# facebookresearch/robust_cvd

Hardware: AMD Instinct MI355X
Metric: GN/LM iterations/sec (and ms/iter) on 300-frame 384x224 video, 1/2/4/8 GPU (higher is better)
Workload: dtype f64

## Files before the change

include/cvd_hip_debug.h:

```cpp
#ifndef CVD_HIP_DEBUG_H
#define CVD_HIP_DEBUG_H

#include "cvd_hip.h"

#ifdef __cplusplus
extern "C" {
#endif

typedef struct cvd_debug_options {
  uint64_t struct_size;
  int32_t force_iterations;
  int32_t force_sharded_path;
  int32_t pcg_lockstep;
  int32_t stall_fused_tail_once;
  int32_t tail_no_row_staging;
  int32_t tail_closes_scalars;
  int32_t asm_force_stage_depth;
  int32_t asm_force_part_units;
} cvd_debug_options;
void cvd_debug_options_default(cvd_debug_options* o);
int32_t cvd_set_debug_options(cvd_handle* h, const cvd_debug_options* o);

int32_t cvd_set_generic_kernels(cvd_handle* h, int32_t enabled);

int32_t cvd_comm_init_local_group(cvd_handle* h, int32_t rank, int32_t world, uint64_t group_key);
int32_t cvd_comm_init_phantom(cvd_handle* h, int32_t rank, int32_t world);

int32_t cvd_block_inverse_debug(cvd_handle* h, int32_t num_blocks, int32_t block_size, const double* a, int32_t variant,
                                float* inverse, int32_t* failed);

int32_t cvd_epipolar_debug(cvd_handle* h, int32_t num_pairs, const int64_t* offsets, const float* loc, double pixel_scale,
                           double threshold_px, int32_t iterations, uint64_t seed, uint8_t* is_static_out,
                           double* fundamental_out, int32_t* best_out, int32_t* counts_out, double* hypotheses_out);
// ... 15 lines not shown
```

robust_cvd_amd/api.py:

```python
import collections
import ctypes as C
import os
import sys

from . import build as _build
from .binding import Binding
from .ctypes_types import OptParams, SolveSummary, XformDesc

_lib = None
_variant = None


class SolverOptions(C.Structure):
    _fields_ = [
        ("struct_size", C.c_uint64),
        ("pcg_relative_tolerance", C.c_double),
        ("pcg_max_iterations", C.c_int32),
        ("verbose", C.c_int32),
        ("coarse_level", C.c_int32),
        ("robust_loss", C.c_int32),
        ("dense_matrix_free", C.c_int32),
        ("block_inverse_variant", C.c_int32),
        ("coarse_dense_max_unknowns", C.c_int32),
        ("coarse_rebuild_excess", C.c_int32),
# ... 14 lines not shown
        ("temporal_weight", C.c_double),
    ]


class DebugOptions(C.Structure):
    _fields_ = [
        ("struct_size", C.c_uint64),
        ("force_iterations", C.c_int32),
        ("force_sharded_path", C.c_int32),
        ("pcg_lockstep", C.c_int32),
        ("stall_fused_tail_once", C.c_int32),
        ("tail_no_row_staging", C.c_int32),
        ("tail_closes_scalars", C.c_int32),
        ("asm_force_stage_depth", C.c_int32),
        ("asm_force_part_units", C.c_int32),
    ]


class ConsistencyDesc(C.Structure):
    _fields_ = [
        ("struct_size", C.c_uint64),
        ("precision", C.c_int32),
        ("num_frames", C.c_int32),
        ("num_pairs", C.c_int32),
        ("height", C.c_int32),
        ("width", C.c_int32),
        ("distance_type", C.c_int32),
        ("have_warp", C.c_int32),
        ("reserved", C.c_int32),
        ("lambda_reprojection", C.c_double),
# ... 1793 lines not shown
        ai = np.zeros((n, n))
        lam = np.zeros(self.num_frames * self.block_size())
        fl = C.c_int32(0)
        dp = lambda x: x.ctypes.data_as(C.POINTER(C.c_double))
        self._check(self._fn("temporal_debug")(self._h, dims, dp(a), dp(ai), dp(lam), C.byref(fl)))
        return {"NT": n, "S": dims[1], "nn": dims[2], "step": dims[3], "Sx": dims[4], "Sy": dims[5], "a_t": a, "a_t_inverse": ai,
                "lam": lam, "failed": fl.value}

    def path_info(self):
        out = (C.c_int32 * 8)()
        self._check(self._fn("path_info")(self._h, out))
        form = {-1: "none", 0: "exact sparse factor", 1: "exact dense inverse", 2: "temporal pose level"}[out[1]]
        return {"pose_graph_level": form, "depth_grid_level": bool(out[2]), "fused_tail": bool(out[3] & 1), "tail_rows_staged": bool(out[3] & 2),
                "product_sums_shares": bool(out[3] & 4), "rz_shares": out[3] >> 8,
                "tail_disabled": bool(out[4]),
                "taps": out[5], "work_items": out[6], "cross_blocks": bool(out[7])}

    def product_launch_debug(self):
        out = (C.c_int32 * 6)()
        self._check(self._fn("product_launch_debug")(self._h, out))
        kind = {-1: "none", 0: "generic list", 1: "fast list", 2: "fast dense", 3: "cross blocks"}[out[3]]
        return {"threads": out[0], "spec": out[1], "kd": out[2], "kind": out[3], "kind_name": kind, "work_items": out[4],
                "num_cu": out[5]}

    def assembly_launch_debug(self):
        import numpy as np
        out = (C.c_int32 * 8)()
        cost = np.zeros(self.num_frames, dtype=np.float64)
        self._check(self._fn("assembly_launch_debug")(self._h, out, cost.ctypes.data_as(C.POINTER(C.c_double))))
        kind = {-1: "none", 0: "generic", 1: "fast list", 2: "fast dense", 3: "dense fold"}[out[3]]
        return {"threads": out[0], "spec": out[1], "kd": out[2], "kind": out[3], "kind_name": kind, "workgroups": out[4],
# ... 15 lines not shown
```

robust_cvd_amd/csrc/cvd_api.hip:

```cpp
#include "cvd_host.h"
#include "cvd_coarse.h"

namespace cvd {

static void poseOptimizationStep(cvd_handle* h, const cvd_opt_params& p, double depthDeformReg) {
  solve(h, p, depthDeformReg, PK_POSE_STEP);
  paramsToPoses(h, p);
}

static void poseOptimization(cvd_handle* h, const cvd_opt_params& p) {
  posesToParams(h);
  h->records.clear();
  int ctfRows = p.ctf_long, ctfCols = p.ctf_short;
  int dsoRows = p.dso_long, dsoCols = p.dso_short;
  if (h->aspect >= 1.f) {
    std::swap(ctfCols, ctfRows);
    std::swap(dsoCols, dsoRows);
  }
  int initGrid[3] = {1, 1, 1};
  if (h->ddesc.depth_type == CVD_DEPTH_GRID)
    for (int i = 0; i < 3; ++i) initGrid[i] = h->ddesc.grid_size[i];
  const int Nval = (h->ddesc.depth_type == CVD_DEPTH_IDENTITY) ? 0 : valueNumParams(h->ddesc.value_xform);
  size_t nDmax = static_cast<size_t>(h->nD());
  if (p.coarse_to_fine && h->ddesc.depth_type != CVD_DEPTH_IDENTITY && p.num_steps > 1)
// ... 243 lines not shown
      h->tableValid = false;
    if (o->constraint_order != h->opt.constraint_order) h->orderGx = h->orderGy = -1;
    h->opt = *o;
  });
}
void cvd_debug_options_default(cvd_debug_options* o) {
  o->struct_size = CVD_STRUCT_STAMP(cvd_debug_options);
  o->force_iterations = 0;
  o->force_sharded_path = 0;
  o->pcg_lockstep = 0;
  o->stall_fused_tail_once = 0;
  o->tail_no_row_staging = 0;
  o->tail_closes_scalars = 0;
  o->asm_force_stage_depth = 0;
  o->asm_force_part_units = 0;
}
int32_t cvd_set_debug_options(cvd_handle* h, const cvd_debug_options* o) {
  CVD_TRY(h, {
    if (o->struct_size != CVD_STRUCT_STAMP(cvd_debug_options))
      throw std::runtime_error("cvd_debug_options: struct_size does not match this library's cvd_hip_debug.h (start from cvd_debug_options_default)");
    if (o->asm_force_stage_depth < 0 || o->asm_force_stage_depth > 3) throw std::runtime_error("asm_force_stage_depth in {0, 1, 2, 3}");
    if (o->asm_force_part_units < 0) throw std::runtime_error("asm_force_part_units >= 0");
    if (o->asm_force_part_units != h->dbg.asm_force_part_units) h->tableValid = false;
    h->dbg = *o;
    h->distForced = h->world == 1 && (h->comm != nullptr || h->localGroup || h->phantom) && o->force_sharded_path != 0;
  });
}
void cvd_comm_unique_id(uint8_t* out128) {
  ncclUniqueId id;
  std::memset(&id, 0, sizeof(id));
// ... 767 lines not shown
      HIP_CHECK(hipStreamSynchronize(s));
      if (failed) *failed = fl;
    }
  });
}
int32_t cvd_path_info(cvd_handle* h, int32_t* out8) {
  CVD_TRY(h, {
    out8[0] = h->coarseOn ? 1 : 0;
    out8[1] = !h->coarseOn ? -1 : (h->coarse.temporalPose ? 2 : (h->coarse.denseMode ? 1 : 0));
    out8[2] = h->temporal.on ? 1 : 0;
    out8[3] = h->lastFusedTail ? (h->tailStageRows ? 3 : 1) : 0;
    if (h->lastFusedTail && h->lastShares) out8[3] |= 4 | (h->lastShareCount << 8);
    out8[4] = h->tailDisabled ? 1 : 0;
    out8[5] = h->lastKD;
    out8[6] = static_cast<int32_t>(h->itemFa.size());
    out8[7] = h->lastCross ? 1 : 0;
  });
}
int32_t cvd_product_launch_debug(cvd_handle* h, int32_t* out6) {
  CVD_TRY(h, {
    for (int i = 0; i < 6; ++i) out6[i] = h->lastProduct[i];
  });
}
int32_t cvd_assembly_launch_debug(cvd_handle* h, int32_t* out8, double* cost_frame) {
  CVD_TRY(h, {
    for (int i = 0; i < 8; ++i) out8[i] = h->lastAssembly[i];
    const size_t F = static_cast<size_t>(h->F);
    if (cost_frame && h->lastAssembly[3] >= 0 && h->dCostFrame.n >= F) {
      h->dCostFrame.download(cost_frame, F, h->stream);
      HIP_CHECK(hipStreamSynchronize(h->stream));
    }
// ... 80 lines not shown
```

robust_cvd_amd/csrc/cvd_eval.hip:

```cpp
#include "cvd_host.h"
#include "cvd_cost.h"
#include "cvd_assembly.h"
#include "cvd_triplets.h"
#include "cvd_dense_walk.h"

namespace cvd {

void launchFrameConsts(Ctx& c, const double* x) {
  launchFrameConsts(c.L, x, c.h->dFc.p, c.h->stream);
  HIP_CHECK(hipGetLastError());
}

void spinStream(hipStream_t s) {
  hipError_t e;
  while ((e = hipStreamQuery(s)) == hipErrorNotReady) {}
  HIP_CHECK(e);
}
void spinEvent(hipEvent_t ev) {
  hipError_t e;
  while ((e = hipEventQuery(ev)) == hipErrorNotReady) {}
  HIP_CHECK(e);
}
void readScalars(Ctx& c) {
  HIP_CHECK(hipMemcpyAsync(c.h->hScal, c.h->dScal.p, S_COUNT * sizeof(double), hipMemcpyDeviceToHost, c.h->stream));
  spinStream(c.h->stream);
}
// ... 264 lines not shown
```

robust_cvd_amd/csrc/cvd_host.h:

```cpp
#pragma once

#include <hip/hip_runtime.h>
#include <hip/hip_ext.h>
#include <rccl/rccl.h>
#include <rocblas/rocblas.h>
#include <rocsolver/rocsolver.h>

#include <algorithm>
#include <array>
#include <atomic>
#include <chrono>
#include <condition_variable>
#include <cmath>
#include <cstdarg>
#include <cstdint>
#include <cstdio>
#include <cstdlib>
#include <cstring>
#include <functional>
#include <limits>
#include <map>
#include <memory>
#include <mutex>
#include <set>
#include <stdexcept>
#include <string>
#include <thread>
#include <tuple>
#include <vector>

#include "../../include/cvd_hip_debug.h"
#include "cvd_kernels.h"
#include "cvd_asm_segments.h"


namespace cvd {

inline std::string fmt(const char* f, ...) {
  char buf[1024];
  va_list ap;
  va_start(ap, f);
  vsnprintf(buf, sizeof(buf), f, ap);
  va_end(ap);
  return buf;
}

#define HIP_CHECK(expr)                                                                          \
  do {                                                                                           \
// ... 278 lines not shown
    DevBuf<TlStep> stepDev;
    hipEvent_t evIn = nullptr, evDone = nullptr;
    bool sidePending = false;
    double* sqPtr = nullptr;
  } temporal;
  hipEvent_t evRebuild[2] = {nullptr, nullptr};
  bool rebuildTimed = false;
  double coarseRebuildMs = 0.0, pcgIterMs = 0.0;
  std::vector<std::pair<int, int>> globalEdges;
  bool haveGlobalEdges = false;
  DevBuf<double> dRegJac;
  DevBuf<unsigned short> dRegCol;
  DevBuf<unsigned char> dRegCnt;
  RegCache regCache{};
  DevBuf<FrameConst> dFc;
  DevBuf<int> dFail;
  DevBuf<unsigned long long> dCount;
  double* hScal = nullptr;
  double* hStage[2] = {nullptr, nullptr};
  size_t hStageN[2] = {0, 0};
  double* hPcg = nullptr;
  hipEvent_t pcgEvent[2] = {nullptr, nullptr};

  cvd_solve_summary summary{};
  std::vector<cvd_iteration_record> records;

  bool lastFusedTail = false, lastCross = false;
  bool lastShares = false;
  int lastShareCount = 0;
  int sharesF = -1, sharesN = -1;
  bool tailStageRows = false;
  int lastKD = 0;
  int lastProduct[6] = {0, 0, 0, -1, 0, 0};
  int lastAssembly[8] = {0, 0, 0, -1, 0, 0, -1, 0};
  bool tailDisabled = false;
  bool forceGeneric = false;

  int timing = 0;
  int timingStride = 1;
  long long timingCounter = 0;
  long long timingCounterKc[16] = {0};
  std::vector<std::pair<hipEvent_t, hipEvent_t>> evPool;
// ... 195 lines not shown
  ~DenseListScope();
};
bool denseModeSupported(const cvd_opt_params& p, const cvd_xform_desc& dd, const cvd_xform_desc& sd, bool haveTriplets, int world,
                        bool normalize);
AsmPanels makePanels(int B, size_t capDoubles, int& panelCap);
void compileTable(cvd_handle* h, const std::vector<int>& range, bool withTriplets = false, bool ignoreStatic = false);
void orderTable(cvd_handle* h, const Layout& L, int KD);
double* pinnedStage(cvd_handle* h, int which, size_t n);
void uploadState(cvd_handle* h, const Layout& L, DevBuf<double>& dst);
void downloadState(cvd_handle* h, const Layout& L, const DevBuf<double>& src);
void buildMask(cvd_handle* h, const Layout& L, const cvd_opt_params& p, ProblemKind kind, const std::vector<int>& range);
void ensureBuffers(Ctx& c);
void refreshMedians(cvd_handle* h);
void launchFrameConsts(const Layout& L, const double* x, FrameConst* fc, hipStream_t s);
void launchFrameConsts(Ctx& c, const double* x);
void launchFlagToBool(int* flag, hipStream_t s);
void launchTlRowsInit(cvd_handle* h, const TlStep* tsp, int NT, int groups, int F, unsigned int* counter, int closeScalars, double tol2,
                      hipStream_t s);
void spinStream(hipStream_t s);
void spinEvent(hipEvent_t ev);
void readScalars(Ctx& c);
void enqueueCost(Ctx& c, const double* x);
double evalCost(Ctx& c, const double* x);
void enqueueStats(Ctx& c);
bool crossScope(cvd_handle* h, const Ctx& c);
CrossPairs crossPairs(cvd_handle* h);
void launchCrossAssemble(Ctx& c, const double* x);
double evalFull(Ctx& c, const double* x, bool withStats = false, bool noReadBack = false);
bool coarseFusedConsumers();
bool fusedExchange(cvd_handle* h, bool withCoarse);
// ... 20 lines not shown
                  double* q, bool withCoarse = false, bool tailFused = false, int sharesIteration = 0);
bool pcgTailScope(Ctx& c, bool coarse, int nThreads, size_t& lds, int& ldsFinish, int& ldsScratch);
struct PcgShares {
  int count = 0;
  int levelShare0 = 0;
  int levelWg0 = 0;
};
bool pcgSharesScope(Ctx& c, bool coarse, PcgShares& sh);
void launchPcgTail(Ctx& c, const double* x, const double* pOld, double* pNew, int useBeta, const double* lam, double* q,
                   bool withCoarse, int nThreads, size_t lds, int ldsFinish, int ldsScratch, double tol2,
                   const PcgShares* shares = nullptr);
void launchPcgClose(Ctx& c, int enqueued);
void launchBlockInverseRaw(cvd_handle* h, const Layout& L, const double* dH, const double* dLam, float* dMinv, int* dFail, int variant,
                           hipStream_t onStream = nullptr);
void launchBlockInverse(Ctx& c, hipStream_t onStream = nullptr);
void launchCoarseSetup(Ctx& c, const double* x, int side = 0);
bool temporalScope(const Ctx& c);
bool temporalPrepare(Ctx& c);
void launchTemporalSetup(Ctx& c, const double* x, int half);
void launchTemporalInit(Ctx& c, bool closeScalars, double tol2);
TlStep temporalStep(cvd_handle* h);
const TlStep* temporalStepDev(cvd_handle* h);
void poseTemporalPlan(cvd_handle* h);
void poseTemporalPrepare(Ctx& c);
void launchPoseTemporalBuild(Ctx& c, hipStream_t s, int* failOut, bool deferInverse = false);
void launchPoseTemporalInit(Ctx& c, double tol2);
const TlStep* poseTemporalStepDev(cvd_handle* h);
void coarseDebug(cvd_handle* h, int32_t* num_unknowns, double* a_c, double* a_c_inverse, int32_t* failed);
int runPcg(Ctx& c, const double* x, const std::function<void()>& tail = nullptr);
bool wantsTriplets(const cvd_opt_params& p, ProblemKind kind);
void bindTriplets(Ctx& c, const cvd_opt_params& p, ProblemKind kind);
void solve(cvd_handle* h, const cvd_opt_params& p, double depthDeformReg, ProblemKind kind);
void evaluate(cvd_handle* h, const cvd_opt_params& p, double depthDeformReg, const double* pose7, double* cost, int32_t* nres,
              double* gradient, double* hdiag, double* hfull);
// ... 115 lines not shown
```

robust_cvd_amd/csrc/cvd_precond.hip:

```cpp
#include "cvd_host.h"
#include "cvd_block_inverse.h"
#include "cvd_coarse.h"
#include "cvd_cross.h"
#include "cvd_dense_walk.h"
#include "cvd_dense_inverse.h"

namespace cvd {

void launchFlagToBool(int* flag, hipStream_t s) { hipLaunchKernelGGL(k_flag_to_bool, dim3(1), dim3(1), 0, s, flag); }

void launchBlockInverseRaw(cvd_handle* h, const Layout& L, const double* dH, const double* dLam, float* dMinv,
                                  int* dFail, int variant, hipStream_t onStream) {
  hipStream_t s = onStream ? onStream : h->stream;
  const int B = L.B;
  if (B > 256) {
    if (onStream) throw std::logic_error("launchBlockInverseRaw: the rocSOLVER route runs on the solver's stream");
    if (!h->rbMain) {
      if (rocblas_create_handle(&h->rbMain) != rocblas_status_success) throw std::runtime_error("rocblas_create_handle failed");
      if (rocblas_set_stream(h->rbMain, s) != rocblas_status_success) throw std::runtime_error("rocblas_set_stream failed");
    }
    const size_t bb = static_cast<size_t>(B) * B, total = bb * L.F;
    h->dInvScratch.ensure(total);
    h->dInvInfo.ensure(2 * static_cast<size_t>(L.F));
    HIP_CHECK(hipMemsetAsync(h->dInvInfo.p, 0, 2 * static_cast<size_t>(L.F) * sizeof(int), s));
// ... 124 lines not shown
  else if (tpw <= 5) CVD_LAUNCH_DINV(5);
  else if (tpw <= 8) CVD_LAUNCH_DINV(8);
  else if (tpw <= 13) CVD_LAUNCH_DINV(13);
  else if (tpw <= 18) CVD_LAUNCH_DINV(18);
  else CVD_LAUNCH_DINV(25);
#undef CVD_LAUNCH_DINV
  HIP_CHECK(hipGetLastError());
}
void launchDenseSpdInversePair(cvd_handle* h, const DinvRequest& a, const DinvRequest& b, hipStream_t s) {
  const DinvPlan Pa = planDenseSpdInverse(h, a.n, a.A, a.out, a.fail, s, a.outValid, a.panelBuf, a.barrierBuf);
  const DinvPlan Pb = planDenseSpdInverse(h, b.n, b.A, b.out, b.fail, s, b.outValid, b.panelBuf, b.barrierBuf);
  const size_t lds = std::max(Pa.lds, Pb.lds);
  bool pair = Pa.tpw <= 2 && Pb.tpw <= 2 && CVD_DETERMINISTIC == 0;
  if (pair) {
    allowLds((k_dense_spd_inverse_pair<2>), lds);
    int perCu = 0;
    HIP_CHECK(hipOccupancyMaxActiveBlocksPerMultiprocessor(&perCu, reinterpret_cast<const void*>(&k_dense_spd_inverse_pair<2>), kDinvNW * 64, lds));
    pair = static_cast<long long>(perCu) * h->numCU >= 2ll * std::max(Pa.job.groups, Pb.job.groups);
  }
  if (!pair) {
    launchDenseSpdInverse(h, a.n, a.A, a.out, a.fail, s, a.outValid, a.panelBuf, a.barrierBuf);
    launchDenseSpdInverse(h, b.n, b.A, b.out, b.fail, s, b.outValid, b.panelBuf, b.barrierBuf);
    return;
  }
  PersistentGate gate(h->device, s);
  hipLaunchKernelGGL((k_dense_spd_inverse_pair<2>), dim3(std::max(Pa.job.groups, Pb.job.groups), 2), dim3(kDinvNW * 64), lds, s, Pa.job, Pb.job);
  HIP_CHECK(hipGetLastError());
}

void launchCoarseSetup(Ctx& c, const double* x, int side) {
  cvd_handle* h = c.h;
  hipStream_t s = side ? h->stream2 : h->stream;
  auto& C = h->coarse;
  const size_t B = c.L.B;
  double* WbOut = side ? C.Wb2.p : C.Wb.p;
  int* failOut = side ? C.fail2.p : C.fail.p;
  FrameConst* fcBuf = side ? h->dFc2.p : h->dFc.p;
  HIP_CHECK(hipMemsetAsync(failOut, 0, sizeof(int), s));
  {
    launchFrameConsts(c.L, x, fcBuf, s);
    HIP_CHECK(hipMemsetAsync(C.edges.p, 0, static_cast<size_t>(std::max(C.nEdges, 1)) * kCBB * sizeof(double), s));
    if (C.sparsified) HIP_CHECK(hipMemsetAsync(C.dropDiag.p, 0, static_cast<size_t>(c.L.F) * kCBB * sizeof(double), s));
    const size_t ldsE = 2 * B * 8 + 2 * sizeof(FrameConst) + 4 * kCBB * 8;
    if (c.cross && !C.sparsified) {
      hipLaunchKernelGGL(k_coarse_edges_cross, dim3(static_cast<unsigned>(h->xFa.size())), dim3(256), 0, s, c.L, crossPairs(h),
                         h->dXBlocks.p, h->dXPairEdge.p, C.edges.p);
    } else if (c.nItems > 0) {
      const bool fast = !h->forceGeneric && c.KS == 0 && fastLoss(c.L) &&
                        c.L.intrOpt != CVD_INTR_SHARED;
      const bool gram = fast && !h->dense && c.KD == 4 && c.L.N == 1 && !C.sparsified && CVD_DETERMINISTIC == 0;
      if (gram) {
        const size_t ldsG = (2 * B + 512 + 4 * 64 * kDwLd) * 8;
        allowLds(k_coarse_edges_mfma, ldsG);
        hipLaunchKernelGGL(k_coarse_edges_mfma, dim3(c.nItems), dim3(256), ldsG, s, c.L, c.T, c.it, x, fcBuf, C.itemEdgeDev.p, C.edges.p);
      } else if (fast) {
// ... 14 lines not shown
          hipLaunchKernelGGL((k_coarse_edges<KD, KS>), dim3(c.nItems), dim3(256), ldsE, s, c.L, c.T, c.it, x, fcBuf,
                             C.itemEdgeDev.p, C.edges.p, C.dropDiag.p);
        });
      }
    }
    HIP_CHECK(hipGetLastError());
    if (h->dist()) {
      const int ct = h->tBegin(KC_COMM_COARSE);
      commAllReduce(h, C.edges.p, static_cast<size_t>(C.nEdges) * kCBB, CT_F64, s);
      if (C.sparsified)
        commAllReduce(h, C.dropDiag.p, static_cast<size_t>(c.L.F) * kCBB, CT_F64, s);
      h->tEnd(ct);
    }
  }
  constexpr double lamPredict = 1.0 / 3.0;
  hipLaunchKernelGGL(k_coarse_diag, dim3(c.L.F), dim3(256), 0, s, c.L, h->dH.p, h->dLam.p, h->dMask.p, C.diag.p,
                     C.modeActive.p, side ? lamPredict : 1.0, C.sparsified ? C.dropDiag.p : nullptr);
  if (h->dist()) {
    const int ct = h->tBegin(KC_COMM_COARSE);
    const size_t chunk = static_cast<size_t>(h->ownChunk()) * kCBB;
    commAllGather(h, C.diag.p + static_cast<size_t>(h->rank) * chunk, C.diag.p, chunk, CT_F64, s);
    h->tEnd(ct);
  }
  if (C.denseMode) {
    if (side) throw std::logic_error("the dense coarse level is built in line");
    if (C.temporalPose) {
      C.denseValid.ensure(1);
      if (!(C.denseReady && C.denseForB == static_cast<int>(c.L.B))) HIP_CHECK(hipMemsetAsync(C.denseValid.p, 0, sizeof(int), s));
      launchPoseTemporalBuild(c, s, failOut, h->temporal.on && !h->dist());
      if (h->dist()) {
        launchFlagToBool(failOut, s);
        const int ct = h->tBegin(KC_COMM_COARSE);
// ... 46 lines not shown
```

robust_cvd_amd/csrc/cvd_setup.hip:

```cpp
#include "cvd_host.h"
#include "cvd_table.h"
#include "cvd_triplets.h"
#include "cvd_dense_walk.h"
#include <rocprim/device/device_segmented_radix_sort.hpp>

namespace cvd {

void launchFrameConsts(const Layout& L, const double* x, FrameConst* fc, hipStream_t s) {
  hipLaunchKernelGGL(k_frame_consts, dim3((L.F + 63) / 64), dim3(64), 0, s, L, x, fc);
}

static void quatToMatrix(const double q[4] , double R[3][3]) {
  for (int c = 0; c < 3; ++c) {
    double v[3] = {0, 0, 0};
    v[c] = 1.0;
    const double uv[3] = {2.0 * (q[1] * v[2] - q[2] * v[1]), 2.0 * (q[2] * v[0] - q[0] * v[2]),
                          2.0 * (q[0] * v[1] - q[1] * v[0])};
    R[0][c] = v[0] + q[3] * uv[0] + (q[1] * uv[2] - q[2] * uv[1]);
    R[1][c] = v[1] + q[3] * uv[1] + (q[2] * uv[0] - q[0] * uv[2]);
    R[2][c] = v[2] + q[3] * uv[2] + (q[0] * uv[1] - q[1] * uv[0]);
  }
}
static void matrixToAngleAxis(const double R[3][3], double aa[3]) {
  double q0, q1, q2, q3;
// ... 1081 lines not shown
  }
  return h->hStage[which];
}

void uploadState(cvd_handle* h, const Layout& L, DevBuf<double>& dst) {
  const size_t nAll = static_cast<size_t>(L.F) * L.B;
  double* x = pinnedStage(h, 1, nAll);
  const int nD = L.nD, nS = L.nS;
  for (int f = 0; f < L.F; ++f) {
    double* xf = &x[static_cast<size_t>(f) * L.B];
    for (int i = 0; i < 7; ++i) xf[i] = h->poseParams[f][i];
    for (int i = 0; i < nD; ++i) xf[7 + i] = h->dparams[static_cast<size_t>(f) * nD + i];
    for (int i = 0; i < nS; ++i) xf[7 + nD + i] = h->sparams[static_cast<size_t>(f) * nS + i];
  }
  dst.upload(x, nAll, h->stream);
  HIP_CHECK(hipStreamSynchronize(h->stream));
}

void downloadState(cvd_handle* h, const Layout& L, const DevBuf<double>& src) {
  const size_t nAll = static_cast<size_t>(L.F) * L.B;
  double* x = pinnedStage(h, 0, nAll);
  src.download(x, nAll, h->stream);
  HIP_CHECK(hipStreamSynchronize(h->stream));
  const int nD = L.nD, nS = L.nS;
  for (int f = 0; f < L.F; ++f) {
    const double* xf = &x[static_cast<size_t>(f) * L.B];
    for (int i = 0; i < 7; ++i) h->poseParams[f][i] = xf[i];
    for (int i = 0; i < nD; ++i) h->dparams[static_cast<size_t>(f) * nD + i] = xf[7 + i];
    for (int i = 0; i < nS; ++i) h->sparams[static_cast<size_t>(f) * nS + i] = xf[7 + nD + i];
  }
// ... 115 lines not shown
```

robust_cvd_amd/csrc/cvd_solve.hip:

```cpp
#include <optional>

#include "cvd_host.h"
#include "cvd_lm.h"
#include "cvd_pcg.h"
#include "cvd_coarse.h"

namespace cvd {

void launchTlRowsInit(cvd_handle* h, const TlStep* tsp, int NT, int groups, int F, unsigned int* counter, int closeScalars, double tol2,
                      hipStream_t s) {
  const size_t lds = static_cast<size_t>(tlRowsLds(NT)) * 8;
  allowLds(k_tl_rows_init, lds);
  hipLaunchKernelGGL(k_tl_rows_init, dim3(groups), dim3(768), lds, s, tsp, F, h->dScal.p, counter, closeScalars, tol2, h->hPcg);
  HIP_CHECK(hipGetLastError());
}

namespace {
struct TailStalled {};
}
static int runPcgAttempt(Ctx& c, const double* x, const std::function<void()>& tail);
int runPcg(Ctx& c, const double* x, const std::function<void()>& tail) {
  const size_t firstTimerSlot = c.h->evUsed;
  try {
    return runPcgAttempt(c, x, tail);
// ... 312 lines not shown
    }
  }
};

void rebuildTemporalLevel(Ctx& c) {
  cvd_handle* h = c.h;
  const int slot = h->tBegin(KC_INVERSE);
  launchTemporalSetup(c, h->dX.p, 0);
  launchTemporalSetup(c, h->dX.p, 1);
  h->tEnd(slot);
}

void buildLevels(Ctx& c, const LevelSchedule::Decision& d, PendingGuard& guard) {
  cvd_handle* h = c.h;
  hipStream_t s = h->stream;
  if (d.inverseAside) {
    HIP_CHECK(hipEventRecord(h->evInvIn, s));
    HIP_CHECK(hipStreamWaitEvent(h->stream3, h->evInvIn, 0));
    launchBlockInverse(c, h->stream3);
    HIP_CHECK(hipEventRecord(h->evInvDone, h->stream3));
    guard.inverseAside = true;
  } else {
    const int slot = h->tBegin(KC_INVERSE);
    launchBlockInverse(c);
    h->tEnd(slot);
  }
  if (d.coarse == LevelSchedule::SIDE_STREAM) {
    h->dFc2.ensure(c.L.F);
    if (h->temporal.on) rebuildTemporalLevel(c);
    HIP_CHECK(hipEventRecord(h->evCoarseIn, s));
    HIP_CHECK(hipStreamWaitEvent(h->stream2, h->evCoarseIn, 0));
    launchCoarseSetup(c, h->dX.p, 1);
    HIP_CHECK(hipEventRecord(h->evCoarseDone, h->stream2));
  } else if (d.coarse == LevelSchedule::IN_LINE) {
    const int slot = h->tBegin(KC_INVERSE);
    const bool measure = h->coarse.denseMode && !h->dist() && h->opt.coarse_rebuild_excess_dense < 0;
    if (measure) {
      if (!h->evRebuild[0]) for (auto& e : h->evRebuild) HIP_CHECK(hipEventCreate(&e));
      HIP_CHECK(hipEventRecord(h->evRebuild[0], s));
    }
    if (h->temporal.on) launchTemporalSetup(c, h->dX.p, 0);
    launchCoarseSetup(c, h->dX.p);
    if (d.inverseAside) {
      HIP_CHECK(hipStreamWaitEvent(s, h->evInvDone, 0));
      guard.inverseAside = false;
    }
    if (h->temporal.on) launchTemporalSetup(c, h->dX.p, 1);
    if (measure) {
      HIP_CHECK(hipEventRecord(h->evRebuild[1], s));
      h->rebuildTimed = true;
    }
    h->tEnd(slot);
  }
  if (d.temporalOnly) rebuildTemporalLevel(c);
}

void installPendingCoarse(cvd_handle* h, LevelSchedule& schedule) {
// ... 27 lines not shown
  h->records.push_back(rec);
  if (tableLine && h->opt.verbose)
    printf("%4d % .6e    % .2e   % .2e   % .2e  % .2e % .2e   %5d\n", rec.iteration, cost, rec.cost_change, gmax, rec.step_norm,
           rec.relative_decrease, radius, rec.linear_iterations);
}

}

void solve(cvd_handle* h, const cvd_opt_params& p, double depthDeformReg, ProblemKind kind) {
  const double t0 = nowSeconds();
  if (h->F <= 0) throw std::runtime_error("no video set");
  if (!h->poseParamsValid) posesToParams(h);
  const std::vector<int> range = rangeOf(p, h->F);
  LevelSchedule schedule;
  PendingGuard guard{h, schedule};
  SetupPhases phase{h->opt.verbose >= 3};
  BoundProblem bound;
  bindProblem(bound, h, p, depthDeformReg, kind, range, BindMode{ true,  true,  true}, phase);
  Ctx& c = bound.c;
  hipStream_t s = h->stream;
  HIP_CHECK(hipMemsetAsync(h->dDx.p, 0, c.n * sizeof(double), s));
  HIP_CHECK(hipMemsetAsync(h->dR.p, 0, c.n * sizeof(double), s));
  HIP_CHECK(hipMemsetAsync(h->dFail.p, 0, sizeof(int), s));

  cvd_solve_summary sum{};
  sum.num_residual_blocks = static_cast<int>((c.L.includeStatic ? h->numValid : 0) + countResidualBlocks(c, range));
  double tEval = 0.0, tLin = 0.0;
  double te = nowSeconds();
  double xCost = evalFull(c, h->dX.p, true, false);
  tEval += nowSeconds() - te;
// ... 29 lines not shown
      ++iteration;
      cvd_iteration_record rec{};
      rec.iteration = iteration;

      double tl = nowSeconds();
      hipLaunchKernelGGL(k_lm_diag, dim3((c.n + 255) / 256), dim3(256), 0, s, c.L, h->dHd.p, h->dScale.p,
                         scaleDone ? 0 : 1, tr.radius, h->dLam.p);
      scaleDone = true;
      buildLevels(c, schedule.decide(levels), guard);
      const double tPcgStart = nowSeconds();
      const int cgIters = runPcg(c, h->dX.p, [&]() {
        enqueueStats(c);
        hipLaunchKernelGGL(k_apply_step, dim3((c.n + 255) / 256), dim3(256), 0, s, c.L, c.boundDepth0, h->dX.p,
                           h->dDx.p, h->dXc.p);
        HIP_CHECK(hipGetLastError());
        enqueueCost(c, h->dXc.p);
      });
      notePcgTime(h, nowSeconds() - tPcgStart, cgIters);
      schedule.afterPcg(cgIters);
      installPendingCoarse(h, schedule);
      tLin += nowSeconds() - tl;
      if (gradPending) {
        gradPending = false;
        gmax = h->hScal[S_GMAX];
        xNorm = std::sqrt(h->hScal[S_XX]);
        h->records.back().gradient_max_norm = gmax;
        if (gradientConverged()) {
          --iteration;
          termination = 0;
          break;
// ... 129 lines not shown
```

robust_cvd_amd/csrc/cvd_temporal.hip:

```cpp
#include "cvd_host.h"
#include "cvd_temporal.h"

namespace cvd {

static int autoCoarse(int g, int wanted) {
  const int s = wanted > 0 ? wanted : (g + 1) / 2;
  return std::min(g, std::max(2, s));
}

bool temporalScope(const Ctx& c) {
  cvd_handle* h = c.h;
  const Layout& L = c.L;
  if (h->opt.temporal_level == 0 || h->forceGeneric || (h->dense && !c.cross) || c.trip) return false;
  if (c.KD != 4 || c.KS != 0 || !fastLoss(L) || L.intrOpt == CVD_INTR_SHARED) return false;
  if (L.N != 1 || L.gz != 1 || L.depthType != CVD_DEPTH_GRID || L.positionRegSqrt > 0.0 || !L.includeStatic) return false;
  if (L.B > 256 || L.nD > 256 || L.gx < 3 || L.gy < 3 || L.nD != L.gx * L.gy) return false;
  const int step = h->opt.temporal_step;
  if (L.F <= 2 * step) return false;
  const int Sx = autoCoarse(L.gx, h->opt.temporal_grid_x), Sy = autoCoarse(L.gy, h->opt.temporal_grid_y);
  if (Sx * Sy > kTlMaxS) return false;
  const int nn = (L.F - 1 + step - 1) / step + 1;
  if (nn * Sx * Sy > kDenseCoarseMaxUnknowns) return false;
  return true;
}
// ... 148 lines not shown
}

TlStep temporalStep(cvd_handle* h) {
  if (h == nullptr || !h->temporal.on || !h->temporal.built)
    return TlStep{nullptr, nullptr, nullptr, nullptr, nullptr, nullptr, nullptr, nullptr, nullptr, 0, 0, 1, 0, 0, 0, 1, kTlSpan, nullptr, 1.0};
  auto& T = h->temporal;
  return TlStep{T.Ainv.p, T.sqPtr, T.rT.p, T.t.p, T.tl.p, T.dotPart.p, T.fail.p, T.elW.p, T.elV.p, T.S, T.nn, T.step, T.NT, T.NT, T.width,
                tlParts(T.nn), kTlSpan, (!h->dist() && T.step <= 32) ? T.rec.p : nullptr,
                h->opt.temporal_weight};
}

const TlStep* temporalStepDev(cvd_handle* h) {
  return (h != nullptr && h->temporal.on && h->temporal.built) ? h->temporal.stepDev.p : nullptr;
}

void launchTemporalSetup(Ctx& c, const double* x, int half) {
  cvd_handle* h = c.h;
  auto& T = h->temporal;
  const Layout& L = c.L;
  const bool side = !h->dist() && h->stream2 != nullptr;
  hipStream_t s = (half == 0 && side) ? h->stream2 : h->stream;
  if (half == 1) {
    if (side && T.sidePending) {
      HIP_CHECK(hipStreamWaitEvent(h->stream, T.evDone, 0));
      T.sidePending = false;
    }
    temporalInverse(c);
    return;
  }
  const TlTables tb = temporalTables(h);
  const size_t SS = static_cast<size_t>(T.S) * T.S;
  FrameConst* fcBuf = h->dFc.p;
  if (side) {
    if (!T.evIn) {
      HIP_CHECK(hipEventCreateWithFlags(&T.evIn, hipEventDisableTiming));
      HIP_CHECK(hipEventCreateWithFlags(&T.evDone, hipEventDisableTiming));
    }
    h->dFc2.ensure(L.F);
    fcBuf = h->dFc2.p;
    HIP_CHECK(hipEventRecord(T.evIn, h->stream));
    HIP_CHECK(hipStreamWaitEvent(s, T.evIn, 0));
  }
  launchFrameConsts(L, x, fcBuf, s);
  const size_t ldsD = static_cast<size_t>(L.nD) * T.S * 8 + static_cast<size_t>(T.width) * T.S * 5 + 16;
  allowLds(k_tl_diag, ldsD);
  hipLaunchKernelGGL(k_tl_diag, dim3(L.F), dim3(256), ldsD, s, L, h->dH.p, h->dLam.p, h->dMask.p, tb, T.Cf.p,
                     h->dist() ? h->ownFirst() : 0, h->dist() ? h->ownCount() : L.F);
  HIP_CHECK(hipGetLastError());
  if (c.cross) {
    if (!h->xFa.empty()) {
      allowLds(k_tl_edges_cross, ldsD);
      hipLaunchKernelGGL(k_tl_edges_cross, dim3(static_cast<unsigned>(h->xFa.size())), dim3(256), ldsD, s, L, h->dXFa.p, h->dXFb.p,
                         h->dXBlocks.p, h->dMask.p, tb, T.E.p);
      hipLaunchKernelGGL(k_tl_reduce, dim3(T.nGroups), dim3(256), 0, s, T.S, T.step, T.gOff.p, T.gItems.p, h->dXFa.p, h->dXFb.p, T.E.p,
                         T.part.p);
      HIP_CHECK(hipGetLastError());
    }
  } else if (c.nItems > 0) {
    const size_t ldsE = 2 * static_cast<size_t>(L.B) * 8 + 2 * sizeof(FrameConst) + SS * 8 + 3 * static_cast<size_t>(L.gx + L.gy) * 4 + 16;
    allowLds(k_tl_edges<false>, ldsE);
    hipLaunchKernelGGL(k_tl_edges<false>, dim3(c.nItems), dim3(256), ldsE, s, L, c.T, c.it, x, fcBuf, h->dMask.p, tb, T.E.p);
    HIP_CHECK(hipGetLastError());
    hipLaunchKernelGGL(k_tl_reduce, dim3(T.nGroups), dim3(256), 0, s, T.S, T.step, T.gOff.p, T.gItems.p, h->dItemFa.p, h->dItemFb.p,
// ... 179 lines not shown
```

Baseline: 359.1.

## Fuse coarse and temporal per-frame diagonal builds; cache frame constants and occupancy query

Adds a single k_level_diag kernel that reads each frame's Hessian block once and produces both the coarse-level diagonal blocks and the temporal-level Cf blocks, replacing the separate k_coarse_diag and k_tl_diag launches on the single-GPU in-line build path. It also tags the frame-constant buffer with a parameter write generation so that repeated launchFrameConsts calls on unchanged parameters are skipped. A third change memoises the occupancy query for the pair inverse kernel. The fused kernel uses LDS double atomics and 1024-thread workgroups, which makes summation order nondeterministic. The cache depends on every parameter write being noted, so a missed write could leave stale constants.

```diff
diff --git a/include/cvd_hip_debug.h b/include/cvd_hip_debug.h
--- a/include/cvd_hip_debug.h
+++ b/include/cvd_hip_debug.h
@@ -17,6 +17,7 @@
   int32_t tail_closes_scalars;
   int32_t asm_force_stage_depth;
   int32_t asm_force_part_units;
+  int32_t level_build_separate;
 } cvd_debug_options;
 void cvd_debug_options_default(cvd_debug_options* o);
 int32_t cvd_set_debug_options(cvd_handle* h, const cvd_debug_options* o);
diff --git a/robust_cvd_amd/api.py b/robust_cvd_amd/api.py
--- a/robust_cvd_amd/api.py
+++ b/robust_cvd_amd/api.py
@@ -52,6 +52,7 @@
         ("tail_closes_scalars", C.c_int32),
         ("asm_force_stage_depth", C.c_int32),
         ("asm_force_part_units", C.c_int32),
+        ("level_build_separate", C.c_int32),
     ]
 
 
@@ -1875,7 +1876,8 @@
         return {"pose_graph_level": form, "depth_grid_level": bool(out[2]), "fused_tail": bool(out[3] & 1), "tail_rows_staged": bool(out[3] & 2),
                 "product_sums_shares": bool(out[3] & 4), "rz_shares": out[3] >> 8,
                 "tail_disabled": bool(out[4]),
-                "taps": out[5], "work_items": out[6], "cross_blocks": bool(out[7])}
+                "taps": out[5], "work_items": out[6], "cross_blocks": bool(out[7] & 1),
+                "level_build_fused": bool(out[7] & 2)}
 
     def product_launch_debug(self):
         out = (C.c_int32 * 6)()
diff --git a/robust_cvd_amd/csrc/cvd_api.hip b/robust_cvd_amd/csrc/cvd_api.hip
--- a/robust_cvd_amd/csrc/cvd_api.hip
+++ b/robust_cvd_amd/csrc/cvd_api.hip
@@ -281,6 +281,7 @@
   o->tail_closes_scalars = 0;
   o->asm_force_stage_depth = 0;
   o->asm_force_part_units = 0;
+  o->level_build_separate = 0;
 }
 int32_t cvd_set_debug_options(cvd_handle* h, const cvd_debug_options* o) {
   CVD_TRY(h, {
@@ -1078,7 +1079,7 @@
     out8[4] = h->tailDisabled ? 1 : 0;
     out8[5] = h->lastKD;
     out8[6] = static_cast<int32_t>(h->itemFa.size());
-    out8[7] = h->lastCross ? 1 : 0;
+    out8[7] = (h->lastCross ? 1 : 0) | (h->lastLevelBuildFused ? 2 : 0);
   });
 }
 int32_t cvd_product_launch_debug(cvd_handle* h, int32_t* out6) {
diff --git a/robust_cvd_amd/csrc/cvd_eval.hip b/robust_cvd_amd/csrc/cvd_eval.hip
--- a/robust_cvd_amd/csrc/cvd_eval.hip
+++ b/robust_cvd_amd/csrc/cvd_eval.hip
@@ -6,10 +6,21 @@
 
 namespace cvd {
 
+static uint64_t frameConstKey(const Layout& L) {
+  uint64_t f;
+  static_assert(sizeof(f) == sizeof(L.vFocal), "vFocal is a double");
+  std::memcpy(&f, &L.vFocal, sizeof(f));
+  return f ^ (static_cast<uint64_t>(L.F) << 40) ^ (static_cast<uint64_t>(L.B) << 20) ^ (static_cast<uint64_t>(L.intrOpt) << 60);
+}
 void launchFrameConsts(Ctx& c, const double* x) {
-  launchFrameConsts(c.L, x, c.h->dFc.p, c.h->stream);
-  HIP_CHECK(hipGetLastError());
-}
+  cvd_handle* h = c.h;
+  const uint64_t key = frameConstKey(c.L);
+  if (h->fcTag.holds(x, h->dFc.p, key)) return;
+  launchFrameConsts(c.L, x, h->dFc.p, h->stream);
+  HIP_CHECK(hipGetLastError());
+  h->fcTag.filled(x, h->dFc.p, key);
+}
+void noteParamsWritten(cvd_handle* h, const double* x) { h->fcTag.wrote(x); }
 
 void spinStream(hipStream_t s) {
   hipError_t e;
diff --git a/robust_cvd_amd/csrc/cvd_fc_tag.h b/robust_cvd_amd/csrc/cvd_fc_tag.h
--- /dev/null
+++ b/robust_cvd_amd/csrc/cvd_fc_tag.h
@@ -0,0 +1,45 @@
+#pragma once
+
+#include <cstdint>
+
+namespace cvd {
+
+struct FrameConstTag {
+  static constexpr int kBufs = 4;
+  struct Buf {
+    const void* p = nullptr;
+    uint64_t gen = 0;
+  };
+  Buf bufs[kBufs];
+  uint64_t clock = 0;
+  const void* x = nullptr;
+  const void* fc = nullptr;
+  uint64_t gen = 0, key = 0;
+
+  uint64_t generationOf(const void* p) const {
+    for (const Buf& b : bufs)
+      if (b.p == p && p != nullptr) return b.gen;
+    return 0;
+  }
+  void wrote(const void* p) {
+    Buf* slot = &bufs[0];
+    for (Buf& b : bufs) {
+      if (b.p == p) { slot = &b; break; }
+      if (b.gen < slot->gen) slot = &b;
+    }
+    slot->p = p;
+    slot->gen = ++clock;
+  }
+  void filled(const void* xp, const void* fcp, uint64_t k) {
+    x = xp;
+    fc = fcp;
+    key = k;
+    gen = generationOf(xp);
+  }
+  bool holds(const void* xp, const void* fcp, uint64_t k) const {
+    return gen != 0 && xp == x && fcp == fc && k == key && generationOf(xp) == gen;
+  }
+  void invalidate() { gen = 0; }
+};
+
+}
diff --git a/robust_cvd_amd/csrc/cvd_host.h b/robust_cvd_amd/csrc/cvd_host.h
--- a/robust_cvd_amd/csrc/cvd_host.h
+++ b/robust_cvd_amd/csrc/cvd_host.h
@@ -32,6 +32,7 @@
 #include "../../include/cvd_hip_debug.h"
 #include "cvd_kernels.h"
 #include "cvd_asm_segments.h"
+#include "cvd_fc_tag.h"
 
 
 namespace cvd {
@@ -340,6 +341,7 @@
   DevBuf<unsigned char> dRegCnt;
   RegCache regCache{};
   DevBuf<FrameConst> dFc;
+  FrameConstTag fcTag;
   DevBuf<int> dFail;
   DevBuf<unsigned long long> dCount;
   double* hScal = nullptr;
@@ -352,6 +354,7 @@
   std::vector<cvd_iteration_record> records;
 
   bool lastFusedTail = false, lastCross = false;
+  bool lastLevelBuildFused = false;
   bool lastShares = false;
   int lastShareCount = 0;
   int sharesF = -1, sharesN = -1;
@@ -577,6 +580,7 @@
 void refreshMedians(cvd_handle* h);
 void launchFrameConsts(const Layout& L, const double* x, FrameConst* fc, hipStream_t s);
 void launchFrameConsts(Ctx& c, const double* x);
+void noteParamsWritten(cvd_handle* h, const double* x);
 void launchFlagToBool(int* flag, hipStream_t s);
 void launchTlRowsInit(cvd_handle* h, const TlStep* tsp, int NT, int groups, int F, unsigned int* counter, int closeScalars, double tol2,
                       hipStream_t s);
@@ -627,10 +631,12 @@
 void launchBlockInverseRaw(cvd_handle* h, const Layout& L, const double* dH, const double* dLam, float* dMinv, int* dFail, int variant,
                            hipStream_t onStream = nullptr);
 void launchBlockInverse(Ctx& c, hipStream_t onStream = nullptr);
-void launchCoarseSetup(Ctx& c, const double* x, int side = 0);
+void launchCoarseSetup(Ctx& c, const double* x, int side = 0, bool frameBlocksDone = false);
 bool temporalScope(const Ctx& c);
 bool temporalPrepare(Ctx& c);
-void launchTemporalSetup(Ctx& c, const double* x, int half);
+void launchTemporalSetup(Ctx& c, const double* x, int half, bool frameBlocksDone = false);
+bool levelBuildFusedScope(const Ctx& c);
+void launchLevelDiag(Ctx& c, hipStream_t s);
 void launchTemporalInit(Ctx& c, bool closeScalars, double tol2);
 TlStep temporalStep(cvd_handle* h);
 const TlStep* temporalStepDev(cvd_handle* h);
diff --git a/robust_cvd_amd/csrc/cvd_level_build.h b/robust_cvd_amd/csrc/cvd_level_build.h
--- /dev/null
+++ b/robust_cvd_amd/csrc/cvd_level_build.h
@@ -0,0 +1,126 @@
+#pragma once
+
+#include "cvd_temporal.h"
+
+namespace cvd {
+
+constexpr int kLevelDiagThreads = 1024;
+constexpr int kLevelDiagRows = 4;
+constexpr int kLevelDiagChunks = 4;
+
+inline __global__ __launch_bounds__(kLevelDiagThreads) void k_level_diag(Layout L, const double* __restrict__ hBlocks,
+                                                                  const double* __restrict__ lam, const double* __restrict__ mask,
+                                                                  TlTables T, double* __restrict__ diagOut,
+                                                                  unsigned char* __restrict__ modeActive, double* __restrict__ Cf) {
+  extern __shared__ __attribute__((aligned(16))) double sm[];
+  __shared__ int anyScale;
+  constexpr int NT = kLevelDiagThreads, NW = NT / 64;
+  const int B = L.B, G = L.nD, S = T.S, Gs = G | 1, f = blockIdx.x, tid = threadIdx.x, lane = tid & 63;
+  const int wave = __builtin_amdgcn_readfirstlane(tid >> 6);
+  double* T1 = sm;
+  double* u = T1 + static_cast<size_t>(S) * Gs;
+  double* red = u + B;
+  float* ew = reinterpret_cast<float*>(red + NW);
+  unsigned char* ev = reinterpret_cast<unsigned char*>(ew + T.width * S);
+  const double* hf = hBlocks + static_cast<size_t>(f) * B * B;
+  const double* lf = lam + static_cast<size_t>(f) * B;
+  const double* mf = mask + static_cast<size_t>(f) * B;
+  double* out = Cf + static_cast<size_t>(f) * S * S;
+  const bool tlOn = mf[7] != 0.0;
+  if (tid == 0) anyScale = 0;
+  for (int r = tid; r < B; r += NT) u[r] = 0.0;
+  if (tlOn) {
+    for (int e = tid; e < S * Gs; e += NT) T1[e] = 0.0;
+    for (int e = tid; e < T.width * S; e += NT) {
+      ew[e] = T.elW[e];
+      ev[e] = T.elV[e];
+    }
+  }
+  __syncthreads();
+  {
+    bool in[kLevelDiagChunks], grid[kLevelDiagChunks];
+    double lv[kLevelDiagChunks], us[kLevelDiagChunks];
+#pragma unroll
+    for (int j = 0; j < kLevelDiagChunks; ++j) {
+      const int c = lane + 64 * j, v = c - 7;
+      in[j] = c < B;
+      grid[j] = in[j] && v >= 0 && v < G;
+      lv[j] = grid[j] ? lf[c] : 0.0;
+      us[j] = 0.0;
+    }
+    const double* col = hf + static_cast<size_t>(7) * B + lane;
+    for (int vp0 = wave; vp0 < G; vp0 += NW * kLevelDiagRows) {
+      double hv[kLevelDiagRows][kLevelDiagChunks];
+#pragma unroll
+      for (int q = 0; q < kLevelDiagRows; ++q) {
+        const int vp = vp0 + NW * q;
+#pragma unroll
+        for (int j = 0; j < kLevelDiagChunks; ++j) hv[q][j] = (vp < G && in[j]) ? col[static_cast<size_t>(vp) * B + 64 * j] : 0.0;
+      }
+#pragma unroll
+      for (int q = 0; q < kLevelDiagRows; ++q) {
+        const int vp = vp0 + NW * q;
+        if (vp >= G) break;
+        const float4 w = T.vW[vp];
+        const unsigned int idx = T.vIdx[vp];
+#pragma unroll
+        for (int j = 0; j < kLevelDiagChunks; ++j) {
+          const int v = lane + 64 * j - 7;
+          const double h = hv[q][j] + (v == vp ? lv[j] : 0.0);
+          us[j] += h;
+          if (tlOn && grid[j]) {
+            if (w.x != 0.f) atomicAdd(&T1[(idx & 255u) * Gs + v], static_cast<double>(w.x) * h);
+            if (w.y != 0.f) atomicAdd(&T1[((idx >> 8) & 255u) * Gs + v], static_cast<double>(w.y) * h);
+            if (w.z != 0.f) atomicAdd(&T1[((idx >> 16) & 255u) * Gs + v], static_cast<double>(w.z) * h);
+            if (w.w != 0.f) atomicAdd(&T1[(idx >> 24) * Gs + v], static_cast<double>(w.w) * h);
+          }
+        }
+      }
+    }
+#pragma unroll
+    for (int j = 0; j < kLevelDiagChunks; ++j)
+      if (in[j]) atomicAdd(&u[lane + 64 * j], us[j]);
+  }
+  __syncthreads();
+  for (int r = 7 + tid; r < 7 + G; r += NT)
+    if (mf[r] != 0.0) anyScale = 1;
+  double s77 = 0.0;
+  for (int v = tid; v < G; v += NT) s77 += u[7 + v];
+  s77 = waveSum(s77);
+  if (lane == 0) red[wave] = s77;
+  __syncthreads();
+  if (tid < kCBB) {
+    const int i = tid / kCB, j = tid % kCB;
+    auto active = [&](int m) -> bool {
+      if (m < 7) return mf[m] != 0.0 && !(m == 6 && L.intrOpt == kIntrShared);
+      return anyScale != 0;
+    };
+    double v;
+    if (i < 7 && j < 7) v = hf[static_cast<size_t>(i) * B + j] + (i == j ? lf[i] : 0.0);
+    else if (i < 7) v = u[i];
+    else if (j < 7) v = u[j];
+    else {
+      v = 0.0;
+      for (int k = 0; k < NW; ++k) v += red[k];
+    }
+    const bool ai = active(i), aj = active(j);
+    if (!(ai && aj)) v = (i == j) ? 1.0 : 0.0;
+    diagOut[static_cast<size_t>(f) * kCBB + tid] = v;
+    if (j == 0) modeActive[f * kCB + i] = ai ? 1 : 0;
+  }
+  if (!tlOn) {
+    for (int e = tid; e < S * S; e += NT) out[e] = 0.0;
+    return;
+  }
+  for (int e = tid; e < S * S; e += NT) {
+    const int s = e / S, sp = e - s * S;
+    double a = 0.0;
+    for (int k = 0; k < T.width; ++k) a += static_cast<double>(ew[k * S + s]) * T1[sp * Gs + ev[k * S + s]];
+    out[e] = a;
+  }
+}
+inline size_t levelDiagLds(const Layout& L, int S, int width) {
+  return (static_cast<size_t>(S) * (L.nD | 1) + static_cast<size_t>(L.B) + kLevelDiagThreads / 64) * 8 + static_cast<size_t>(width) * S * 5 + 16;
+}
+
+}
diff --git a/robust_cvd_amd/csrc/cvd_precond.hip b/robust_cvd_amd/csrc/cvd_precond.hip
--- a/robust_cvd_amd/csrc/cvd_precond.hip
+++ b/robust_cvd_amd/csrc/cvd_precond.hip
@@ -162,8 +162,19 @@
   bool pair = Pa.tpw <= 2 && Pb.tpw <= 2 && CVD_DETERMINISTIC == 0;
   if (pair) {
     allowLds((k_dense_spd_inverse_pair<2>), lds);
+    static std::mutex occMutex;
+    static std::map<std::pair<int, size_t>, int> occ;
     int perCu = 0;
-    HIP_CHECK(hipOccupancyMaxActiveBlocksPerMultiprocessor(&perCu, reinterpret_cast<const void*>(&k_dense_spd_inverse_pair<2>), kDinvNW * 64, lds));
+    {
+      std::lock_guard<std::mutex> lock(occMutex);
+      auto it = occ.find({h->device, lds});
+      if (it == occ.end()) {
+        HIP_CHECK(hipOccupancyMaxActiveBlocksPerMultiprocessor(&perCu, reinterpret_cast<const void*>(&k_dense_spd_inverse_pair<2>), kDinvNW * 64, lds));
+        occ[{h->device, lds}] = perCu;
+      } else {
+        perCu = it->second;
+      }
+    }
     pair = static_cast<long long>(perCu) * h->numCU >= 2ll * std::max(Pa.job.groups, Pb.job.groups);
   }
   if (!pair) {
@@ -176,7 +187,7 @@
   HIP_CHECK(hipGetLastError());
 }
 
-void launchCoarseSetup(Ctx& c, const double* x, int side) {
+void launchCoarseSetup(Ctx& c, const double* x, int side, bool frameBlocksDone) {
   cvd_handle* h = c.h;
   hipStream_t s = side ? h->stream2 : h->stream;
   auto& C = h->coarse;
@@ -185,8 +196,10 @@
   int* failOut = side ? C.fail2.p : C.fail.p;
   FrameConst* fcBuf = side ? h->dFc2.p : h->dFc.p;
   HIP_CHECK(hipMemsetAsync(failOut, 0, sizeof(int), s));
+  if (frameBlocksDone && (side || h->dist())) throw std::logic_error("the fused level build is an in-line build on one GPU");
   {
-    launchFrameConsts(c.L, x, fcBuf, s);
+    if (side) launchFrameConsts(c.L, x, fcBuf, s);
+    else launchFrameConsts(c, x);
     HIP_CHECK(hipMemsetAsync(C.edges.p, 0, static_cast<size_t>(std::max(C.nEdges, 1)) * kCBB * sizeof(double), s));
     if (C.sparsified) HIP_CHECK(hipMemsetAsync(C.dropDiag.p, 0, static_cast<size_t>(c.L.F) * kCBB * sizeof(double), s));
     const size_t ldsE = 2 * B * 8 + 2 * sizeof(FrameConst) + 4 * kCBB * 8;
@@ -231,8 +244,10 @@
     }
   }
   constexpr double lamPredict = 1.0 / 3.0;
-  hipLaunchKernelGGL(k_coarse_diag, dim3(c.L.F), dim3(256), 0, s, c.L, h->dH.p, h->dLam.p, h->dMask.p, C.diag.p,
-                     C.modeActive.p, side ? lamPredict : 1.0, C.sparsified ? C.dropDiag.p : nullptr);
+  if (!frameBlocksDone) {
+    hipLaunchKernelGGL(k_coarse_diag, dim3(c.L.F), dim3(256), 0, s, c.L, h->dH.p, h->dLam.p, h->dMask.p, C.diag.p,
+                       C.modeActive.p, side ? lamPredict : 1.0, C.sparsified ? C.dropDiag.p : nullptr);
+  }
   if (h->dist()) {
     const int ct = h->tBegin(KC_COMM_COARSE);
     const size_t chunk = static_cast<size_t>(h->ownChunk()) * kCBB;
diff --git a/robust_cvd_amd/csrc/cvd_setup.hip b/robust_cvd_amd/csrc/cvd_setup.hip
--- a/robust_cvd_amd/csrc/cvd_setup.hip
+++ b/robust_cvd_amd/csrc/cvd_setup.hip
@@ -1119,6 +1119,7 @@
     for (int i = 0; i < nS; ++i) xf[7 + nD + i] = h->sparams[static_cast<size_t>(f) * nS + i];
   }
   dst.upload(x, nAll, h->stream);
+  noteParamsWritten(h, dst.p);
   HIP_CHECK(hipStreamSynchronize(h->stream));
 }
 
diff --git a/robust_cvd_amd/csrc/cvd_solve.hip b/robust_cvd_amd/csrc/cvd_solve.hip
--- a/robust_cvd_amd/csrc/cvd_solve.hip
+++ b/robust_cvd_amd/csrc/cvd_solve.hip
@@ -350,8 +350,26 @@
 void buildLevels(Ctx& c, const LevelSchedule::Decision& d, PendingGuard& guard) {
   cvd_handle* h = c.h;
   hipStream_t s = h->stream;
+  const bool inLine = d.coarse == LevelSchedule::IN_LINE;
+  const bool fused = inLine && levelBuildFusedScope(c);
+  const bool measure = inLine && h->coarse.denseMode && !h->dist() && h->opt.coarse_rebuild_excess_dense < 0;
+  if (inLine) h->lastLevelBuildFused = fused;
+  auto rebuildStarts = [&]() -> int {
+    const int slot = h->tBegin(KC_INVERSE);
+    if (measure) {
+      if (!h->evRebuild[0]) for (auto& e : h->evRebuild) HIP_CHECK(hipEventCreate(&e));
+      HIP_CHECK(hipEventRecord(h->evRebuild[0], s));
+    }
+    return slot;
+  };
+  int rebuildSlot = -1;
+  auto fusedBlocks = [&]() {
+    rebuildSlot = rebuildStarts();
+    launchLevelDiag(c, s);
+  };
   if (d.inverseAside) {
     HIP_CHECK(hipEventRecord(h->evInvIn, s));
+    if (fused) fusedBlocks();
     HIP_CHECK(hipStreamWaitEvent(h->stream3, h->evInvIn, 0));
     launchBlockInverse(c, h->stream3);
     HIP_CHECK(hipEventRecord(h->evInvDone, h->stream3));
@@ -360,6 +378,7 @@
     const int slot = h->tBegin(KC_INVERSE);
     launchBlockInverse(c);
     h->tEnd(slot);
+    if (fused) fusedBlocks();
   }
   if (d.coarse == LevelSchedule::SIDE_STREAM) {
     h->dFc2.ensure(c.L.F);
@@ -369,14 +388,9 @@
     launchCoarseSetup(c, h->dX.p, 1);
     HIP_CHECK(hipEventRecord(h->evCoarseDone, h->stream2));
   } else if (d.coarse == LevelSchedule::IN_LINE) {
-    const int slot = h->tBegin(KC_INVERSE);
-    const bool measure = h->coarse.denseMode && !h->dist() && h->opt.coarse_rebuild_excess_dense < 0;
-    if (measure) {
-      if (!h->evRebuild[0]) for (auto& e : h->evRebuild) HIP_CHECK(hipEventCreate(&e));
-      HIP_CHECK(hipEventRecord(h->evRebuild[0], s));
-    }
-    if (h->temporal.on) launchTemporalSetup(c, h->dX.p, 0);
-    launchCoarseSetup(c, h->dX.p);
+    const int slot = fused ? rebuildSlot : rebuildStarts();
+    if (h->temporal.on) launchTemporalSetup(c, h->dX.p, 0, fused);
+    launchCoarseSetup(c, h->dX.p, 0, fused);
     if (d.inverseAside) {
       HIP_CHECK(hipStreamWaitEvent(s, h->evInvDone, 0));
       guard.inverseAside = false;
@@ -434,6 +448,7 @@
   const std::vector<int> range = rangeOf(p, h->F);
   LevelSchedule schedule;
   PendingGuard guard{h, schedule};
+  h->lastLevelBuildFused = false;
   SetupPhases phase{h->opt.verbose >= 3};
   BoundProblem bound;
   bindProblem(bound, h, p, depthDeformReg, kind, range, BindMode{ true,  true,  true}, phase);
@@ -493,6 +508,7 @@
         hipLaunchKernelGGL(k_apply_step, dim3((c.n + 255) / 256), dim3(256), 0, s, c.L, c.boundDepth0, h->dX.p,
                            h->dDx.p, h->dXc.p);
         HIP_CHECK(hipGetLastError());
+        noteParamsWritten(h, h->dXc.p);
         enqueueCost(c, h->dXc.p);
       });
       notePcgTime(h, nowSeconds() - tPcgStart, cgIters);
diff --git a/robust_cvd_amd/csrc/cvd_temporal.hip b/robust_cvd_amd/csrc/cvd_temporal.hip
--- a/robust_cvd_amd/csrc/cvd_temporal.hip
+++ b/robust_cvd_amd/csrc/cvd_temporal.hip
@@ -1,5 +1,6 @@
 #include "cvd_host.h"
 #include "cvd_temporal.h"
+#include "cvd_level_build.h"
 
 namespace cvd {
 
@@ -186,7 +187,23 @@
   return (h != nullptr && h->temporal.on && h->temporal.built) ? h->temporal.stepDev.p : nullptr;
 }
 
-void launchTemporalSetup(Ctx& c, const double* x, int half) {
+bool levelBuildFusedScope(const Ctx& c) {
+  const cvd_handle* h = c.h;
+  return CVD_DETERMINISTIC == 0 && !h->dbg.level_build_separate && h->coarseOn && h->temporal.on && !h->dist() && !h->dense && !c.cross &&
+         !h->coarse.sparsified && c.L.B <= 64 * kLevelDiagChunks;
+}
+void launchLevelDiag(Ctx& c, hipStream_t s) {
+  cvd_handle* h = c.h;
+  auto& C = h->coarse;
+  auto& T = h->temporal;
+  const size_t lds = levelDiagLds(c.L, T.S, T.width);
+  allowLds(k_level_diag, lds);
+  hipLaunchKernelGGL(k_level_diag, dim3(c.L.F), dim3(kLevelDiagThreads), lds, s, c.L, h->dH.p, h->dLam.p, h->dMask.p, temporalTables(h),
+                     C.diag.p, C.modeActive.p, T.Cf.p);
+  HIP_CHECK(hipGetLastError());
+}
+
+void launchTemporalSetup(Ctx& c, const double* x, int half, bool frameBlocksDone) {
   cvd_handle* h = c.h;
   auto& T = h->temporal;
   const Layout& L = c.L;
@@ -213,12 +230,15 @@
     HIP_CHECK(hipEventRecord(T.evIn, h->stream));
     HIP_CHECK(hipStreamWaitEvent(s, T.evIn, 0));
   }
-  launchFrameConsts(L, x, fcBuf, s);
   const size_t ldsD = static_cast<size_t>(L.nD) * T.S * 8 + static_cast<size_t>(T.width) * T.S * 5 + 16;
-  allowLds(k_tl_diag, ldsD);
-  hipLaunchKernelGGL(k_tl_diag, dim3(L.F), dim3(256), ldsD, s, L, h->dH.p, h->dLam.p, h->dMask.p, tb, T.Cf.p,
-                     h->dist() ? h->ownFirst() : 0, h->dist() ? h->ownCount() : L.F);
-  HIP_CHECK(hipGetLastError());
+  if (fcBuf == h->dFc.p) launchFrameConsts(c, x);
+  else launchFrameConsts(L, x, fcBuf, s);
+  if (!frameBlocksDone) {
+    allowLds(k_tl_diag, ldsD);
+    hipLaunchKernelGGL(k_tl_diag, dim3(L.F), dim3(256), ldsD, s, L, h->dH.p, h->dLam.p, h->dMask.p, tb, T.Cf.p,
+                       h->dist() ? h->ownFirst() : 0, h->dist() ? h->ownCount() : L.F);
+    HIP_CHECK(hipGetLastError());
+  }
   if (c.cross) {
     if (!h->xFa.empty()) {
       allowLds(k_tl_edges_cross, ldsD);
```

After: 363.5, median of 6. 1.2% higher.
